# backtato/ai-video-detector

Hardware: AMD Instinct MI355X
Metric: sampled frames/sec analysed (1080p30 60 s clip, 2 fps sampling) (higher is better)
Workload: dtype u8 pixels; f32/f64 Farneback (cv2's own types); 1 GPU; BASELINE.json configs[1]: 1080p30 60 s clip, 2 fps sampling, one clip per GPU per step; frames_per_clip=120, height=1080, width=1920, clips_in_flight_per_gpu=3, fb_mode=fast+rerun, fb_wide160=2, parallelism=single GPU, rccl_ranks_seen=1

## Files before the change

### ai-video-detector_amd/csrc/avd_farneback.hip

```cpp
#include "avd_internal.h"
#include "avd_fb_device.h"

#pragma clang fp contract(off)

namespace {

constexpr int S = AVD_SMALL;

template <int K>
struct PyrGeo {
    static constexpr int WL = S >> K;
    static constexpr int NC = K == 0 ? S : 2 * WL;
    static constexpr int OFF = K == 0 ? 0 : (1 << K) / 2 - 1;
    static constexpr int TR = K >= 2 ? 4 : 8;
    static constexpr int TILES = WL / TR;
    static constexpr int KS = K == 3 ? 19 : (K == 2 ? 9 : 3), HALF = KS / 2;
    static constexpr int SROWS = K == 0 ? TR + 2 * HALF : ((TR - 1) << K) + 2 + 2 * HALF;
    static constexpr int PADX = 12, PS = S + 2 * PADX;
    static constexpr int SRC_BYTES = SROWS * PS, LDS_BYTES = SRC_BYTES + SROWS * NC * 4;
};
constexpr int cmax(int a, int b) { return a > b ? a : b; }
constexpr int cgcd(int a, int b) { return b == 0 ? a : cgcd(b, a % b); }

template <int PR>
// ... 22 lines not shown
    constexpr int WL = G::WL, NC = G::NC, OFF = G::OFF, TR = G::TR, KS = G::KS, HALF = G::HALF, SROWS = G::SROWS;
    constexpr int PADX = G::PADX, PS = G::PS;
    uint8_t (*src)[PS] = reinterpret_cast<uint8_t (*)[PS]>(lds);
    float (*rowf)[NC] = reinterpret_cast<float (*)[NC]>(lds + G::SRC_BYTES);
    const int tiles = WL / TR;
    const int f = blk / tiles, t = blk - f * tiles;
    const int tid = threadIdx.x;
    const int dy0 = t * TR;
    const int y_first = (K == 0 ? dy0 : (dy0 << K) + OFF) - HALF;
    const uint8_t* img = small + (int64_t)f * AVD_NPIX;
    const bool cmp = K == 1 && pairdiff != nullptr && f + 1 < n;
    int differs = 0;
    for (int it = tid; it < SROWS * (S / 4); it += 256) {
        const int r = it / (S / 4), c4 = it - r * (S / 4);
        const int y = reflect101(y_first + r, S);
        const unsigned v = reinterpret_cast<const unsigned*>(img + y * S)[c4];
        reinterpret_cast<unsigned*>(src[r] + PADX)[c4] = v;
        if (K == 1 && cmp) differs |= v != reinterpret_cast<const unsigned*>(img + AVD_NPIX + y * S)[c4];
    }
    for (int it = tid; it < SROWS * 2 * HALF; it += 256) {
        const int r = it / (2 * HALF), i = it - r * (2 * HALF);
        const uint8_t* g = img + reflect101(y_first + r, S) * S;
        if (i < HALF) src[r][PADX - 1 - i] = g[1 + i];
        else src[r][PADX + S + (i - HALF)] = g[S - 2 - (i - HALF)];
    }
    if (K == 1 && cmp) {
        const int any = __syncthreads_or(differs);
        if (tid == 0) pairdiff[f * tiles + t] = any;
    } else
        __syncthreads();
    float kw[KS];
#pragma unroll
    for (int q = 0; q < KS; q++) kw[q] = C->gk[K][q];
    if (KS == 3) {
        static_assert(KS != 3 || NC == S, "the 3-tap scales filter whole rows");
        using W = PyrWalk<S / 4>;
        typedef float f4 __attribute__((ext_vector_type(4)));
        const unsigned* wp0[W::PER]; f4* dst0[W::PER]; int r0[W::PER];
        {
            int r, c4;
            W::first(tid, r, c4);
#pragma unroll
            for (int i = 0; i < W::PER; i++) {
                r0[i] = r;
                wp0[i] = reinterpret_cast<const unsigned*>(src[r] + PADX + 4 * c4);
                dst0[i] = reinterpret_cast<f4*>(&rowf[r][4 * c4]);
                W::next(r, c4);
            }
        }
        for (int sb = 0; sb < SROWS; sb += W::SG) {
#pragma unroll
            for (int i = 0; i < W::PER; i++) {
                if (256 * i >= SROWS * (S / 4) || r0[i] + sb >= SROWS) continue;
                const unsigned* wp = wp0[i] + sb * (PS / 4);
                const unsigned pw = wp[-1], cwd = wp[0], nw = wp[1];
                const float b[6] = {(float)(pw >> 24), (float)(cwd & 0xFFu), (float)((cwd >> 8) & 0xFFu), (float)((cwd >> 16) & 0xFFu),
                                    (float)(cwd >> 24), (float)(nw & 0xFFu)};
                f4 o;
#pragma unroll
                for (int e = 0; e < 4; e++) o[e] = __builtin_fmaf(b[e + 1], kw[1], (b[e] + b[e + 2]) * kw[0]);
                dst0[i][sb * (NC / 4)] = o;
            }
        }
    } else {
        using W = PyrWalk<NC>;
        constexpr int NW = (KS + 3) / 4;
        const unsigned* wp0[W::PER]; float* dst0[W::PER]; int r0[W::PER], sh0[W::PER];
        {
            int r, j;
            W::first(tid, r, j);
#pragma unroll
            for (int i = 0; i < W::PER; i++) {
                const int x = K == 0 ? j : ((j >> 1) << K) + OFF + (j & 1);
                const int base = PADX + x - HALF;
                r0[i] = r; sh0[i] = base & 3;
                wp0[i] = reinterpret_cast<const unsigned*>(src[r] + (base & ~3));
                dst0[i] = &rowf[r][j];
                W::next(r, j);
            }
        }
        for (int sb = 0; sb < SROWS; sb += W::SG) {
#pragma unroll
            for (int i = 0; i < W::PER; i++) {
                if (256 * i >= SROWS * NC || r0[i] + sb >= SROWS) continue;
                const unsigned* wp = wp0[i] + sb * (PS / 4);
                unsigned d[NW + 1];
#pragma unroll
                for (int q = 0; q <= NW; q++) d[q] = wp[q];
                float v = 0.f;
#pragma unroll
                for (int q = 0; q < NW; q++) {
                    const unsigned wv = __builtin_amdgcn_alignbyte(d[q + 1], d[q], sh0[i]);
#pragma unroll
                    for (int e = 0; e < 4; e++)
                        if (q * 4 + e < KS) v = __builtin_fmaf((float)((wv >> (8 * e)) & 0xFFu), kw[q * 4 + e], v);
                }
                dst0[i][sb * NC] = v;
            }
        }
    }
    __syncthreads();
    auto colf = [&](const float* c) {
        float sacc = __builtin_fmaf(c[0], kw[HALF], 0.f);
#pragma unroll
        for (int k = 1; k <= HALF; k++) sacc = __builtin_fmaf(c[k * NC] + c[-k * NC], kw[HALF + k], sacc);
        return sacc;
    };
    {
        using W = PyrWalk<WL>;
        float* out = I + ((int64_t)f * WL + dy0) * WL;
        int dyl, dx;
        W::first(tid, dyl, dx);
#pragma unroll
        for (int i = 0; i < W::PER; i++) {
            if (256 * i < TR * WL) {
                for (int y = dyl; y < TR; y += W::SG) {
                    float o;
                    if (K == 0) {
                        o = colf(&rowf[y + HALF][dx]);
                    } else {
                        const float* c = &rowf[(y << K) + HALF][2 * dx];
                        const float p00 = colf(c), p01 = colf(c + 1);
                        const float p10 = colf(c + NC), p11 = colf(c + NC + 1);
                        o = ((p00 + p01) + (p10 + p11)) * 0.25f;
                    }
                    out[y * WL + dx] = o;
                }
            }
            W::next(dyl, dx);
        }
    }
}

__global__ __launch_bounds__(256) void k_pyramid_all(const uint8_t* __restrict__ small, int n, const FbConsts* __restrict__ C,
                                                    float* __restrict__ I0, float* __restrict__ I1, float* __restrict__ I2,
                                                    float* __restrict__ I3, int* __restrict__ flags, int* __restrict__ pairdiff)
{
    static_assert(PyrGeo<1>::TILES == kPairDiffTiles, "avd_fbfast.hip reads one word per 160-px tile");
    __shared__ __align__(16) char lds[kPyrLds];
    if (flags && (int)(blockIdx.x * 256 + threadIdx.x) < n - 1) flags[blockIdx.x * 256 + threadIdx.x] = 0;
    const int n3 = n * PyrGeo<3>::TILES, n2 = n * PyrGeo<2>::TILES, n1 = n * PyrGeo<1>::TILES;
    int b = blockIdx.x;
    if (b < n3) { pyramid_body<3>(lds, b, small, C, I3); return; }
    b -= n3;
    if (b < n2) { pyramid_body<2>(lds, b, small, C, I2); return; }
    b -= n2;
    if (b < n1) { pyramid_body<1>(lds, b, small, C, I1, n, pairdiff); return; }
    if (I0) pyramid_body<0>(lds, b - n1, small, C, I0);
}

struct PolyPtrs { const float* I[AVD_FB_LEVELS]; float* R[AVD_FB_LEVELS]; const uint8_t* small; };

constexpr int kPolyRows = 16;

template <bool FOLD>
__device__ __forceinline__ void polyexp_rows320(const float* __restrict__ img, const uint8_t* __restrict__ small, float* __restrict__ out, int y0,
                                                const FbConsts* __restrict__ C, float (*rowb)[3][S + 80], float (*outb)[S * 5])
{
    constexpr int w = S, h = S;
    const int x = threadIdx.x;
    const int xs = x - 1 < 0 ? 0 : (x - 1 > w - 4 ? w - 4 : x - 1);
    const int shl = ((x == 0 ? 1 : x - 1) - xs) * 8, shc = (x - xs) * 8, shr = ((x == w - 1 ? w - 2 : x + 1) - xs) * 8;
    const float kx0 = C->gk[0][0], kx1 = C->gk[0][1], kx2 = C->gk[0][2];
    struct __attribute__((packed, aligned(1))) U4 { unsigned v; };
    auto hb = [&](int srow) __attribute__((always_inline)) {
        const int sr = srow < 0 ? -srow : (srow > h - 1 ? 2 * (h - 1) - srow : srow);
        const unsigned wd = reinterpret_cast<const U4*>(small + sr * w + xs)->v;
        const float l = (float)((wd >> shl) & 0xFFu), c = (float)((wd >> shc) & 0xFFu), r = (float)((wd >> shr) & 0xFFu);
        return __builtin_fmaf(c, kx1, (l + r) * kx0);
    };
    float hm = 0.f, h0 = 0.f, hp = 0.f;
    int rcur = -1000;
    auto blurred = [&](int r) __attribute__((always_inline)) {
        if (r != rcur) {
            if (r == rcur + 1) { hm = h0; h0 = hp; hp = hb(r + 1); }
            else { hm = hb(r - 1); h0 = hb(r); hp = hb(r + 1); }
            rcur = r;
        }
        return __builtin_fmaf(hp + hm, kx2, __builtin_fmaf(h0, kx1, 0.f));
    };
    auto pixel = [&](int r) __attribute__((always_inline)) { return FOLD ? blurred(r) : img[r * w + x]; };
    typedef float f4 __attribute__((ext_vector_type(4)));
    typedef float f2 __attribute__((ext_vector_type(2)));
    float g[6], xg[6], xxg[6];
    double gd[6], xxgd[6];
#pragma unroll
    for (int q = 0; q <= 5; q++) { g[q] = C->g[5 + q]; xg[q] = C->xg[5 + q]; xxg[q] = C->xxg[5 + q]; gd[q] = (double)g[q]; xxgd[q] = (double)xxg[q]; }
    const double ig11 = C->ig11, ig03 = C->ig03, ig33 = C->ig33, ig55 = C->ig55;
    float win[11 + kPolyRows];
#pragma unroll
    for (int q = 0; q < 10; q++) win[q] = pixel(min(max(y0 - 5 + q, 0), h - 1));
#pragma unroll
    for (int i = 0; i < kPolyRows; i++) {
        const int y = y0 + i, par = i & 1;
        win[i + 10] = pixel(min(y + 5, h - 1));
        {
            f2 t02 = f2{win[i + 5] * g[0], 0.f};
            float t1 = 0.f;
#pragma unroll
            for (int q = 1; q <= 5; q++) {
                const float a = win[i + 5 - q], bb = win[i + 5 + q];
                const float p = a + bb;
                t02 = t02 + f2{g[q], xxg[q]} * f2{p, p};
                t1 = t1 + xg[q] * (bb - a);
            }
            float* r0s = rowb[par][0]; float* r1s = rowb[par][1]; float* r2s = rowb[par][2];
            const float t0 = t02.x, t2 = t02.y;
            r0s[x + 5] = t0; r1s[x + 5] = t1; r2s[x + 5] = t2;
            if (x == 0)
                for (int q = 0; q < 5; q++) { r0s[q] = t0; r1s[q] = t1; r2s[q] = t2; }
            if (x == w - 1)
                for (int q = 0; q < 5; q++) { r0s[w + 5 + q] = t0; r1s[w + 5 + q] = t1; r2s[w + 5 + q] = t2; }
        }
        __syncthreads();
        if (i > 0) {
            f4* dst = reinterpret_cast<f4*>(out + (int64_t)(y - 1) * w * 5);
            const f4* srcv = reinterpret_cast<const f4*>(outb[par ^ 1]);
            __builtin_nontemporal_store(srcv[x], dst + x);
            if (x < S * 5 / 4 - 320) __builtin_nontemporal_store(srcv[x + 320], dst + x + 320);
        }
        const float* r0 = rowb[par][0] + x + 5; const float* r1 = rowb[par][1] + x + 5; const float* r2 = rowb[par][2] + x + 5;
        double b1 = (double)(r0[0] * g[0]), b2 = 0, b3 = (double)(r1[0] * g[0]), b4 = 0, b5 = (double)(r2[0] * g[0]), b6 = 0;
#pragma unroll
        for (int q = 1; q <= 5; q++) {
            const float r0p = r0[q], r0m = r0[-q], r1p = r1[q], r1m = r1[-q], r2p = r2[q], r2m = r2[-q];
            const double tg = (double)(r0p + r0m);
            b1 = __builtin_fma(tg, gd[q], b1);
            b4 = __builtin_fma(tg, xxgd[q], b4);
            b2 += (double)((r0p - r0m) * xg[q]);
            b3 += (double)((r1p + r1m) * g[q]);
            b6 += (double)((r1p - r1m) * xg[q]);
            b5 += (double)((r2p + r2m) * g[q]);
        }
        float* o = outb[par] + x * 5;
        o[0] = (float)(b3 * ig11);
        o[1] = (float)(b2 * ig11);
        o[2] = (float)(b1 * ig03 + b5 * ig33);
        o[3] = (float)(b1 * ig03 + b4 * ig33);
        o[4] = (float)(b6 * ig55);
    }
    __syncthreads();
    {
        f4* dst = reinterpret_cast<f4*>(out + (int64_t)(y0 + kPolyRows - 1) * w * 5);
        const f4* srcv = reinterpret_cast<const f4*>(outb[(kPolyRows - 1) & 1]);
        __builtin_nontemporal_store(srcv[x], dst + x);
        if (x < S * 5 / 4 - 320) __builtin_nontemporal_store(srcv[x + 320], dst + x + 320);
    }
}

__global__ __launch_bounds__(320) void k_polyexp_all(PolyPtrs P, int n, const FbConsts* __restrict__ C)
{
    __shared__ float rowb[2][3][S + 80];
    __shared__ __align__(16) float outbb[2][S * 5];
    float (*row)[S + 80] = rowb[0];
    float* outb = outbb[0];
    {
        const int wgs0 = n * (S / kPolyRows), cnt0 = ((wgs0 + 7) >> 3) << 3;
        if ((int)blockIdx.x < cnt0) {
            const int per = cnt0 >> 3, lid = ((int)blockIdx.x & 7) * per + ((int)blockIdx.x >> 3);
            if (lid >= wgs0) return;
            const int f = lid / (S / kPolyRows), y0 = (lid - f * (S / kPolyRows)) * kPolyRows;
            if (P.small) polyexp_rows320<true>(nullptr, P.small + (int64_t)f * S * S, P.R[0] + (int64_t)f * S * S * 5, y0, C, rowb, outbb);
            else polyexp_rows320<false>(P.I[0] + (int64_t)f * S * S, nullptr, P.R[0] + (int64_t)f * S * S * 5, y0, C, rowb, outbb);
            return;
        }
    }
    int b = (int)blockIdx.x - ((((n * (S / kPolyRows)) + 7) >> 3) << 3), k = 1;
    for (; k < AVD_FB_LEVELS; k++) {
        const int cnt = ((n * (S >> (2 * k)) + 7) >> 3) << 3;
        if (b < cnt) break;
        b -= cnt;
    }
    if (k >= AVD_FB_LEVELS) return;
    const int wgs = n * (S >> (2 * k));
    const int per = ((wgs + 7) >> 3), lid = (b & 7) * per + (b >> 3);
    if (lid >= wgs) return;
    const int w = S >> k, h = w;
    const int wgs_per_frame = h >> k;
    const int f = lid / wgs_per_frame, y0 = (lid - f * wgs_per_frame) << k;
    const int tid = threadIdx.x;
    const int sr = tid / w, x = tid - sr * w;
    const int y = y0 + sr;
    const float* img = P.I[k] + (int64_t)f * w * h;
    const float* g = C->g + 5; const float* xg = C->xg + 5; const float* xxg = C->xxg + 5;
    const int pitch = w + 10;
    float* r0s = row[0] + sr * pitch; float* r1s = row[1] + sr * pitch; float* r2s = row[2] + sr * pitch;
    {
        float t0 = img[y * w + x] * g[0], t1 = 0.f, t2 = 0.f;
#pragma unroll
        for (int q = 1; q <= 5; q++) {
            const float a = img[max(y - q, 0) * w + x], bb = img[min(y + q, h - 1) * w + x];
            const float p = a + bb;
            t0 = t0 + g[q] * p;
            t1 = t1 + xg[q] * (bb - a);
            t2 = t2 + xxg[q] * p;
        }
        r0s[x + 5] = t0; r1s[x + 5] = t1; r2s[x + 5] = t2;
        if (x == 0)
            for (int q = 0; q < 5; q++) { r0s[q] = t0; r1s[q] = t1; r2s[q] = t2; }
        if (x == w - 1)
            for (int q = 0; q < 5; q++) { r0s[w + 5 + q] = t0; r1s[w + 5 + q] = t1; r2s[w + 5 + q] = t2; }
    }
    __syncthreads();
    const float* r0 = r0s + x + 5; const float* r1 = r1s + x + 5; const float* r2 = r2s + x + 5;
    double b1 = (double)(r0[0] * g[0]), b2 = 0, b3 = (double)(r1[0] * g[0]), b4 = 0,
           b5 = (double)(r2[0] * g[0]), b6 = 0;
#pragma unroll
    for (int q = 1; q <= 5; q++) {
        const double tg = (double)(r0[q] + r0[-q]);
        b1 = __builtin_fma(tg, (double)g[q], b1);
        b4 = __builtin_fma(tg, (double)xxg[q], b4);
        b2 += (double)((r0[q] - r0[-q]) * xg[q]);
        b3 += (double)((r1[q] + r1[-q]) * g[q]);
        b6 += (double)((r1[q] - r1[-q]) * xg[q]);
        b5 += (double)((r2[q] + r2[-q]) * g[q]);
    }
    float* o = outb + tid * 5;
    o[0] = (float)(b3 * C->ig11);
    o[1] = (float)(b2 * C->ig11);
    o[2] = (float)(b1 * C->ig03 + b5 * C->ig33);
    o[3] = (float)(b1 * C->ig03 + b4 * C->ig33);
    o[4] = (float)(b6 * C->ig55);
    __syncthreads();
    typedef float f4 __attribute__((ext_vector_type(4)));
    f4* dst = reinterpret_cast<f4*>(P.R[k] + ((int64_t)f * w * h + (int64_t)y0 * w) * 5);
    const f4* srcv = reinterpret_cast<const f4*>(outb);
    __builtin_nontemporal_store(srcv[tid], dst + tid);
    if (tid < S * 5 / 4 - 320) __builtin_nontemporal_store(srcv[tid + 320], dst + tid + 320);
}

template <int W>
__global__ __launch_bounds__(256) void k_flow_up(const float* __restrict__ prev, float* __restrict__ flow, int npairs, const int* __restrict__ plist)
{
    constexpr int H = W, PW = W / 2, PH = H / 2, Q = W / 4;
    const int gid = blockIdx.x * 256 + threadIdx.x;
    if (gid >= npairs * 2 * H * Q) return;
    const int q = gid % Q;
    const int dy = (gid / Q) % H;
    int pc = gid / (Q * H);
    if (plist) pc = plist[pc >> 1] * 2 + (pc & 1);
    const float* src = prev + (int64_t)pc * PW * PH;
    float fy = dy * 0.5f - 0.25f;
    const int sy = floor_f(fy);
    fy -= sy;
    const float* r0 = src + clampi(sy, 0, PH - 1) * PW;
    const float* r1 = src + clampi(sy + 1, 0, PH - 1) * PW;
    const float b0 = 1.f - fy, b1 = fy;
    float o[4];
#pragma unroll
    for (int i = 0; i < 4; i++) {
        const int dx = q * 4 + i;
        float fx = dx * 0.5f - 0.25f;
        int sx = floor_f(fx);
        fx -= sx;
        if (sx < 0) { fx = 0; sx = 0; }
        bool edge = false;
        if (sx + 1 >= PW) { edge = true; if (sx >= PW - 1) { fx = 0; sx = PW - 1; } }
        const int x1 = min(sx + 1, PW - 1);
        const float a0 = 1.f - fx, a1 = fx;
        float d0, d1;
        if (edge) { d0 = r0[sx] * 1.f; d1 = r1[sx] * 1.f; }
        else { d0 = r0[sx] * a0 + r0[x1] * a1; d1 = r1[sx] * a0 + r1[x1] * a1; }
        o[i] = (d0 * b0 + d1 * b1) * 2.f;
    }
    *reinterpret_cast<float4*>(flow + ((int64_t)pc * H + dy) * W + q * 4) = make_float4(o[0], o[1], o[2], o[3]);
}

constexpr int kChunk = 8192;
constexpr int kNChunk = (AVD_NPIX + kChunk - 1) / kChunk;

__device__ __forceinline__ float chunk_total(const float* part)
{
    float t = part[0];
#pragma unroll
    for (int i = 1; i < kNChunk; i++) t += part[i];
    return t;
}

__global__ __launch_bounds__(512) void k_stats_pair(const float* __restrict__ mag, float* __restrict__ stats, const int* __restrict__ plist)
{
    __shared__ float wpart[kNChunk][8];
    __shared__ float ctot[kNChunk];
    const int p = plist ? plist[blockIdx.x] : (int)blockIdx.x, tid = threadIdx.x;
    const int l = tid >> 3, wave = tid >> 6;
    const bool in_last = l < ((AVD_NPIX - (kNChunk - 1) * kChunk) >> 7);
    const float* src = mag + (int64_t)p * AVD_NPIX + l * 128 + (tid & 7);
    float v[kNChunk][16];
#pragma unroll
    for (int c = 0; c < kNChunk; c++)
#pragma unroll
        for (int k = 0; k < 16; k++) v[c][k] = (c < kNChunk - 1 || in_last) ? src[c * kChunk + 8 * k] : 0.f;
    float total[2];
#pragma unroll
    for (int pass = 0; pass < 2; pass++) {
#pragma unroll
        for (int c = 0; c < kNChunk; c++) {
            float r = v[c][0];
#pragma unroll
            for (int k = 1; k < 16; k++) r += v[c][k];
#pragma unroll
            for (int d = 1; d < 64; d <<= 1) r = r + __shfl_down(r, d);
            if ((tid & 63) == 0) wpart[c][wave] = r;
        }
        __syncthreads();
        if (tid < kNChunk) {
            const float* w = wpart[tid];
            ctot[tid] = tid < kNChunk - 1 ? ((w[0] + w[1]) + (w[2] + w[3])) + ((w[4] + w[5]) + (w[6] + w[7])) : (w[0] + w[1]) + (w[2] + w[3]);
        }
        __syncthreads();
        total[pass] = chunk_total(ctot);
        if (pass == 0) {
            const float mean32 = total[0] / (float)AVD_NPIX;
#pragma unroll
            for (int c = 0; c < kNChunk; c++)
#pragma unroll
                for (int k = 0; k < 16; k++) { const float d = v[c][k] - mean32; v[c][k] = d * d; }
            __syncthreads();
        }
    }
    if (tid == 0) {
        stats[2 * p] = (float)((double)total[0] / (double)AVD_NPIX);
        stats[2 * p + 1] = (float)((double)total[1] / (double)AVD_NPIX);
    }
}

__global__ void k_mag(const float* __restrict__ flow, float* __restrict__ mag, int64_t total4, const int* __restrict__ plist)
{
    const int64_t gid = (int64_t)blockIdx.x * 256 + threadIdx.x;
    if (gid >= total4) return;
    const int64_t ps = gid / (AVD_NPIX / 4), i = gid - ps * (AVD_NPIX / 4);
    const int64_t p = plist ? plist[ps] : ps;
    const float4 fx = reinterpret_cast<const float4*>(flow + p * 2 * AVD_NPIX)[i], fy = reinterpret_cast<const float4*>(flow + (p * 2 + 1) * AVD_NPIX)[i];
    float4 m;
    m.x = sqrtf(fx.x * fx.x + fy.x * fy.x);
    m.y = sqrtf(fx.y * fx.y + fy.y * fy.y);
    m.z = sqrtf(fx.z * fx.z + fy.z * fy.z);
    m.w = sqrtf(fx.w * fx.w + fy.w * fy.w);
    reinterpret_cast<float4*>(mag + p * AVD_NPIX)[i] = m;
}

__global__ void k_flow_interleave(const float* __restrict__ flow, float* __restrict__ out, int64_t total)
{
    const int64_t gid = (int64_t)blockIdx.x * 256 + threadIdx.x;
    if (gid >= total) return;
    const int64_t p = gid / AVD_NPIX, i = gid - p * AVD_NPIX;
    out[gid * 2] = flow[p * 2 * AVD_NPIX + i];
    out[gid * 2 + 1] = flow[(p * 2 + 1) * AVD_NPIX + i];
}

template <typename... A>
inline void launch1d(void (*k)(A...), int64_t items, int block, hipStream_t s, A... args)
{
    const int grid = (int)((items + block - 1) / block);
    if (grid > 0) hipLaunchKernelGGL(k, dim3(grid), dim3(block), 0, s, args...);
}

constexpr int kLevelId[AVD_FB_LEVELS] = {AVD_K_LEVEL320, AVD_K_LEVEL160, AVD_K_LEVEL80, AVD_K_LEVEL40};
constexpr int kFlowUpId[AVD_FB_LEVELS - 1] = {AVD_K_FLOWUP320, AVD_K_FLOWUP160, AVD_K_FLOWUP80};

void pyramid_and_polyexp(avd_ctx* ctx, const uint8_t* d_small, int n)
{
    Workspace& ws = ctx->ws;
    const FbConsts* C = ctx->d_fbc;
    const bool fold = ctx->fb_fold_blur != 0;
    const int wgs = n * ((fold ? 0 : PyrGeo<0>::TILES) + PyrGeo<1>::TILES + PyrGeo<2>::TILES + PyrGeo<3>::TILES);
    kmark(ctx, AVD_K_PYRAMID);
    hipLaunchKernelGGL(k_pyramid_all, dim3(wgs), dim3(256), 0, ctx->stream, d_small, n, C, fold ? nullptr : ws.d_pyr[0].p, ws.d_pyr[1].p, ws.d_pyr[2].p,
                       ws.d_pyr[3].p, ws.d_fbflags.p, ws.d_pairdiff.p);
    PolyPtrs P;
    P.small = fold ? d_small : nullptr;
    int grid = ((n * (S / kPolyRows) + 7) >> 3) << 3;
    for (int k = 0; k < AVD_FB_LEVELS; k++) {
        P.I[k] = ws.d_pyr[k]; P.R[k] = ws.d_poly[k];
        if (k > 0) grid += ((n * (S >> (2 * k)) + 7) >> 3) << 3;
    }
    kmark(ctx, AVD_K_POLYEXP);
    hipLaunchKernelGGL(k_polyexp_all, dim3(grid), dim3(320), 0, ctx->stream, P, n, C);
}

void flow_up_level(hipStream_t stream, int k, const float* prev, float* flow, int np, const int* plist)
{
    fb_dispatch_width(S >> k, [&](auto wc) {
        constexpr int W = decltype(wc)::value;
        if constexpr (W > S / 8) launch1d(k_flow_up<W>, (int64_t)np * 2 * W * (W / 4), 256, stream, prev, flow, np, plist);
    });
}

int exact_levels(avd_ctx* ctx, int np, int fused_mask, FbTwoScratch scratch, const int* plist)
{
    Workspace& ws = ctx->ws;
    const hipStream_t stream = ctx->stream;
    const bool rerun = plist != nullptr;
    float* const flow0 = rerun ? const_cast<float*>(ws.flow_res[0]) : ws.d_flow[0].p;
    if (rerun) kmark(ctx, AVD_K_RERUN);
    for (int k = AVD_FB_LEVELS - 1; k >= 0; k--) {
        const int w = S >> k;
        const bool coarsest = k == AVD_FB_LEVELS - 1, fused = (fused_mask >> k) & 1;
        float* flow = k == 0 ? flow0 : ws.d_flow[k].p;
        if (coarsest) {
            if (!fused && rerun) { ctx->err = "exact re-run: the coarsest level runs the fused kernel (it needs no cleared flow)"; return AVD_ERR_ARG; }
            if (!fused) HIP_TRY(ctx, hipMemsetAsync(flow, 0, sizeof(float) * 2 * w * w * np, stream));
        } else {
            if (!rerun) kmark(ctx, kFlowUpId[k]);
            flow_up_level(stream, k, ws.d_flow[k + 1], flow, np, plist);
        }
        if (!rerun) { ws.flow_res[k] = flow; kmark(ctx, kLevelId[k]); }
        const bool marks = !rerun && k == 0;
        if (fused) {
            stage_mark(ctx, marks);
            if (int e = launch_fb_level(ctx, stream, w, ws.d_poly[k], flow, np, 3, coarsest, plist)) return e;
            stage_mark(ctx, marks);
        } else {
            for (int it = 0; it < 3; it++)
                if (int e = launch_fb_two(ctx, stream, w, ws.d_poly[k], flow, scratch, np, plist, marks)) return e;
        }
    }
    return 0;
}

int fast_levels(avd_ctx* ctx, int np)
{
    Workspace& ws = ctx->ws;
    const hipStream_t stream = ctx->stream;
    const int fold = ctx->fb_fold_up;
    int* flags = ctx->fb_rerun ? ws.d_fbflags.p : nullptr;
    const int* pairdiff = ctx->fb_rerun ? ws.d_pairdiff.p : nullptr;
    for (int k = AVD_FB_LEVELS - 1; k >= 0; k--) {
        const int w = S >> k;
        const bool coarsest = k == AVD_FB_LEVELS - 1, three = (k == 2 || k == 3) && (fold & 4);
        float *a = ws.d_flow[k], *b = ws.d_flow2[k];
        const float* prev = coarsest ? nullptr : ws.flow_res[k + 1];
        const bool chain = (k == 0 && (fold & 1)) || (k == 1 && ctx->fb_fold_up160 && ctx->fb_wide160_used);
        const FbFlowFrom from = coarsest ? FbFlowFrom::zero : chain ? FbFlowFrom::chain
                                : ((k == 1 || k == 2) && (fold & 2)) ? FbFlowFrom::prologue : FbFlowFrom::level;
        if (from == FbFlowFrom::level) {
            kmark(ctx, kFlowUpId[k]);
            flow_up_level(stream, k, prev, a, np, nullptr);
        }
        const bool from_prev = from == FbFlowFrom::chain || from == FbFlowFrom::prologue;
        kmark(ctx, kLevelId[k]);
        stage_mark(ctx, k == 0);
        if (three) {
            const FbFastLaunch L{3, from, from_prev ? prev : a, b, a, nullptr, flags, pairdiff};
            if (int e = launch_fb_fast(ctx, stream, w, ws.d_poly[k], L, np)) return e;
            a = b;
        } else {
            for (int it = 0; it < 3; it++) {
                float* mag = (k == 0 && it == 2) ? ws.d_mag.p : nullptr;
                const FbFastLaunch L{1, it == 0 ? from : FbFlowFrom::level, it == 0 && from_prev ? prev : a, b, a, mag, flags, pairdiff};
                if (int e = launch_fb_fast(ctx, stream, w, ws.d_poly[k], L, np)) return e;
                float* t = a; a = b; b = t;
            }
        }
        stage_mark(ctx, k == 0);
        ws.flow_res[k] = a;
    }
    return 0;
}

void flow_tail(avd_ctx* ctx, const float* flow, bool with_mag, int m, const int* plist, int np_chunk)
{
    Workspace& ws = ctx->ws;
    const hipStream_t stream = ctx->stream;
    if (with_mag) launch1d(k_mag, (int64_t)m * (AVD_NPIX / 4), 256, stream, flow, ws.d_mag.p, (int64_t)m * (AVD_NPIX / 4), plist);
    hipLaunchKernelGGL(k_stats_pair, dim3(m), dim3(512), 0, stream, (const float*)ws.d_mag, ws.d_stats.p, plist);
    if (!ws.no_flow_il && ws.d_flow_il)
        launch1d(k_flow_interleave, (int64_t)np_chunk * AVD_NPIX, 256, stream, flow, ws.d_flow_il.p, (int64_t)np_chunk * AVD_NPIX);
}

}

int launch_farneback(avd_ctx* ctx, const uint8_t* d_small, int n)
{
    if (n < 2) return 0;
    Workspace& ws = ctx->ws;
    if (ctx->profiling) ctx->kern_ev_used = 0;
    const bool fast = ctx->fb_mode == 1;
    ws.mag_valid = fast;
    pyramid_and_polyexp(ctx, d_small, n);
    if (int e = fast ? fast_levels(ctx, n - 1) : exact_levels(ctx, n - 1, ctx->fb_fused, {ws.d_vs, ws.d_vs0}, nullptr)) return e;
    HIP_TRY(ctx, hipGetLastError());
    return 0;
}

int launch_farneback_rerun(avd_ctx* ctx, const int* h_list, int m, int np_chunk)
{
    if (m <= 0) return 0;
    Workspace& ws = ctx->ws;
    if (m > ws.fb_cap) { ctx->err = "re-run list longer than the chunk"; return AVD_ERR_ARG; }
    if (int e = ws.d_rlist.reserve(ctx, (size_t)ws.fb_cap)) return e;
    const int fused_mask = m <= kRerunTwoKernelMax ? (ctx->fb_rerun_fused & 0xF) : 0xF;
    if (fused_mask != 0xF) {
        const FbTwoScratchSize sz = fb_two_scratch_size(kRerunTwoKernelMax);
        if (int e = ws.d_vs0_rerun.reserve(ctx, sz.vs0)) return e;
        if (int e = ws.d_vs_rerun.reserve(ctx, sz.vs)) return e;
    }
    HIP_TRY(ctx, hipMemcpyAsync(ws.d_rlist, h_list, sizeof(int) * m, hipMemcpyHostToDevice, ctx->stream));
    if (int e = exact_levels(ctx, m, fused_mask, {ws.d_vs_rerun, ws.d_vs0_rerun}, ws.d_rlist)) return e;
    flow_tail(ctx, ws.flow_res[0], true, m, ws.d_rlist, np_chunk);
    HIP_TRY(ctx, hipGetLastError());
    return 0;
}

int launch_flow_stats(avd_ctx* ctx, int n)
{
    if (n < 2) return 0;
    Workspace& ws = ctx->ws;
    kmark(ctx, AVD_K_STATS);
    flow_tail(ctx, ws.flow_res[0] ? ws.flow_res[0] : ws.d_flow[0].p, !ws.mag_valid, n - 1, nullptr, n - 1);
    HIP_TRY(ctx, hipGetLastError());
    return 0;
}
```

### ai-video-detector_amd/csrc/avd_internal.h

```cpp
#pragma once
#include <hip/hip_runtime.h>
#include <stdint.h>
#include <mutex>
#include <string>
#include <type_traits>
#include <vector>
#include "../../include/avd.h"
#include "avd_ingest_clip.h"

#define AVD_FB_LEVELS 4
#define AVD_NPIX (AVD_SMALL * AVD_SMALL)
constexpr int kPairDiffTiles = 20;

#define HIP_TRY(ctx, expr)                                                         \
    do {                                                                           \
        hipError_t e__ = (expr);                                                   \
        if (e__ != hipSuccess) {                                                   \
            (ctx)->err = std::string(#expr) + ": " + hipGetErrorString(e__);       \
            return AVD_ERR_DEVICE;                                                 \
        }                                                                          \
    } while (0)

struct LinearTab {
    std::vector<int> x0, x1, y0, y1;
    std::vector<short> a0, a1, b0, b1;
};
void build_linear_tab(int src_h, int src_w, int dst_h, int dst_w, LinearTab& t);

struct AreaAxis {
    std::vector<int> begin, count;
    std::vector<float> w_first, w_mid, w_last;
};
struct AreaTab {
    AreaAxis x, y;
    int fast;
    int iscale_x, iscale_y;
};
int build_area_tab(int src_h, int src_w, int dst_h, int dst_w, AreaTab& t);

struct FbConsts {
    float g[11], xg[11], xxg[11];
    double ig11, ig03, ig33, ig55;
    float gk[AVD_FB_LEVELS][19];
    int gksize[AVD_FB_LEVELS];
};
void build_fb_consts(FbConsts& c);

struct YuvConsts { int cy, crv, cbu, cgu, cgv, c0, kr, kb, kg, bias, ntab; };
void build_yuv_consts(YuvConsts& c, bool full_range);
void yuv_index_window(const YuvConsts& c, int& lo, int& hi);

struct LinTap { short i0, i1, w0, w1; };

struct PreParams {
    const LinTap *lxt, *lyt;
    const int* band_dy;
    const int *ax_begin, *ax_count;
    const float *ax_first, *ax_mid, *ax_last;
    int area_fast;
    int area_x_uniform4;
    int h, w, rows_per_band, nbands, pitch;
    int64_t row_stride, frame_stride;
};

struct HashParams {
    const int *ay_begin, *ay_count;
    const float *ay_first, *ay_mid, *ay_last;
    int area_fast, fast_area, fast_simd_w;
    int h;
};

struct BandPlan { int rows_per_band, pitch, ni; };
BandPlan band_plan(int w);
enum IngestKernel { kIngestBgrScalar = 0, kIngestBgrVec16, kIngestBgrStaged, kIngestNv12Scalar, kIngestNv12Tables, kIngestI420Scalar, kIngestI420Tables,
                    kIngestNv12Strip, kIngestI420Strip, kIngestPx32Scalar, kIngestPx32Vec16, kIngestRgbpScalar, kIngestRgbpVec16, kIngestRgbpStaged,
                    kIngestYuyvScalar, kIngestYuyvTables, kIngestI422Scalar, kIngestI422Tables, kIngestNv16Scalar, kIngestNv16Tables,
                    kIngestP010Scalar, kIngestP010Tables, kIngestI010Scalar, kIngestI010Tables, kIngestP010Strip, kIngestI010Strip };
static_assert(kIngestP010Scalar == 20 && kIngestI010Strip == 25, "the ids include/avd.h lists");
struct IngestPlan { int h, w, rows_per_band, nbands, pitch, ni, lds_bytes, kernel; };
static_assert(sizeof(IngestPlan) == 8 * sizeof(int), "avd_debug_fetch hands the struct out as int32[8]");
struct IngestRecord {
    IngestPlan plan{};
    int launched = 0;
    int32_t rotate = 0;
    int32_t range = 0;
    int32_t format = 0;
    int32_t list[2] = {0, 0};
    int64_t stage_copies = -1;
    int64_t stage_bytes = -1;
};
enum CnnShape { kCnnFolded = 0, kCnn128x128, kCnn256x64, kCnn256x128, kCnn256x256, kCnnStem, kCnnConv3Expand, kCnnSlab3Expand };
constexpr int kCnnConvs = 53;
constexpr int kCnnTapImage = 1, kCnnTapConv0 = 2, kCnnTapMaxPool = kCnnTapConv0 + kCnnConvs, kCnnTapPooled = kCnnTapMaxPool + 1;
constexpr int kLapSlots = 8;

struct avd_ctx;
template <typename T, bool kPinned>
struct Buf {
    T* p = nullptr;
    size_t cap = 0;
    Buf() = default;
    Buf(const Buf&) = delete;
    Buf& operator=(const Buf&) = delete;
    Buf(Buf&& o) noexcept : p(o.p), cap(o.cap) { o.p = nullptr; o.cap = 0; }
    Buf& operator=(Buf&& o) noexcept
    {
        if (this != &o) { reset(); p = o.p; cap = o.cap; o.p = nullptr; o.cap = 0; }
        return *this;
    }
    ~Buf() { reset(); }
    void reset()
    {
        if (p) { if (kPinned) (void)hipHostFree(p); else (void)hipFree(p); }
        p = nullptr; cap = 0;
    }
    int reserve(avd_ctx* ctx, size_t count);
    operator T*() const { return p; }
};
template <typename T> using DevBuf = Buf<T, false>;
template <typename T> using PinBuf = Buf<T, true>;

constexpr int kGeomCache = 4;
struct Geom {
    int h = 0, w = 0;
    DevBuf<uint8_t> d_tables;
    PreParams pre{};
    HashParams hsh{};
    unsigned long long stamp = 0;
};

struct Workspace {
    int cap_n = 0;
    Geom geoms[kGeomCache];
    unsigned long long geom_clock = 0;
    int f0 = 0; size_t rowbuf_off = 0, lappart_off = 0;
    int fb_cap = 0;
    DevBuf<int> d_clipstart; PinBuf<int> h_clipstart;
    DevBuf<uint8_t> d_stage;
    DevBuf<const uint8_t*> d_ftab; PinBuf<const uint8_t*> h_ftab;
    DevBuf<uint8_t> d_small;
    DevBuf<float> d_rowbuf;
    DevBuf<uint8_t> d_area;
    DevBuf<uint8_t> d_hash;
    DevBuf<unsigned long long> d_lap;
    DevBuf<long long> d_lap_part;
    PreParams pre{};
    HashParams hsh{};
    DevBuf<float> d_pyr[AVD_FB_LEVELS];
    DevBuf<float> d_poly[AVD_FB_LEVELS];
    DevBuf<float> d_flow[AVD_FB_LEVELS];
    DevBuf<float> d_flow2[AVD_FB_LEVELS];
    const float* flow_res[AVD_FB_LEVELS] = {};
    DevBuf<float> d_mag;
    int mag_valid = 0;
    DevBuf<int> d_fbflags;
    DevBuf<int> d_pairdiff;
    DevBuf<int> d_rlist;
    PinBuf<int> h_rlist;
    DevBuf<double> d_vs_rerun, d_vs0_rerun;
    DevBuf<double> d_vs;
    DevBuf<double> d_vs0;
    DevBuf<float> d_flow_il;
    int no_flow_il = 0;
    DevBuf<float> d_stats;
    DevBuf<avd_frame_record> d_rec;
    PinBuf<avd_frame_record> h_rec;
    DevBuf<uint16_t> d_vit_patches;
    DevBuf<float> d_vit_tokens;
    DevBuf<double> d_audio_tab; int audio_win = 0, audio_last = 0;
    DevBuf<double> d_audio_buf;
    DevBuf<avd_audio_window> d_audio_out;
    DevBuf<uint16_t> d_cnn_act[4], d_cnn_img;
    DevBuf<float> d_cnn_pool, d_cnn_logits; int cnn_frames = 0;
    DevBuf<uint16_t> d_cnn_tap;
    int cnn_tap_asked = 0, cnn_tap_point = 0;
    size_t cnn_tap_rows = 0, cnn_tap_bytes = 0;
    int cnn_tap_c = 0;
};

struct Weights {
    DevBuf<uint16_t> d_cnn_w; DevBuf<float> d_cnn_b;
    std::vector<size_t> cnn_w_off; size_t cnn_fc_off = 0;
    DevBuf<uint16_t> d_vit_w; DevBuf<float> d_vit_bias; int vit_has_bias = 0;
};

struct avd_ctx {
    int device = 0;
    int num_cus = 256;
    hipStream_t stream = nullptr;
    hipEvent_t ev0 = nullptr, ev1 = nullptr;
    hipEvent_t ev_in = nullptr;
    avd_frame_record* pending_out = nullptr;
    int pending_n = 0;
    hipEvent_t stage_ev[5] = {};
    hipEvent_t kern_ev[12] = {};
    int kern_ev_used = 0;
    int profiling = 0;
// ... 127 lines not shown
```

### ai-video-detector_amd/csrc/avd_tables.cpp

```cpp
#include <cfloat>
#include <climits>
#include <cmath>
#include <cstring>
#include "avd_internal.h"

namespace {

inline int round_half_even(double v) { return (int)std::nearbyint(v); }
inline int round_half_even(float v) { return (int)std::nearbyintf(v); }
inline int floor_i(float v) { int i = (int)v; return i - (i > v); }
inline int floor_i(double v) { int i = (int)v; return i - (i > v); }
inline int ceil_i(double v) { int i = (int)v; return i + (i < v); }
inline short to_q11(float v) {
    int i = round_half_even(v * 2048.f);
    return (short)std::min(32767, std::max(-32768, i));
}
inline int clamp_idx(int v, int n) { return v < 0 ? 0 : (v >= n ? n - 1 : v); }

void linear_axis(int src, int dst, bool snap_weights_at_edges, std::vector<int>& i0,
                 std::vector<int>& i1, std::vector<short>& w0, std::vector<short>& w1)
{
    const double scale = 1. / ((double)dst / src);
    i0.resize(dst); i1.resize(dst); w0.resize(dst); w1.resize(dst);
    for (int d = 0; d < dst; d++) {
        float f = (float)((d + 0.5) * scale - 0.5);
        int s = floor_i(f);
        f -= s;
        if (snap_weights_at_edges) {
            if (s < 0) { f = 0; s = 0; }
            if (s >= src - 1) { f = 0; s = src - 1; }
        }
        w0[d] = to_q11(1.f - f);
        w1[d] = to_q11(f);
        i0[d] = clamp_idx(s, src);
        i1[d] = clamp_idx(s + 1, src);
    }
}

void area_axis(int src, int dst, double scale, AreaAxis& ax)
{
    ax.begin.assign(dst, 0); ax.count.assign(dst, 0);
    ax.w_first.assign(dst, 0.f); ax.w_mid.assign(dst, 0.f); ax.w_last.assign(dst, 0.f);
    for (int d = 0; d < dst; d++) {
        const double lo = d * scale, hi = lo + scale;
        const double cell = std::min(scale, src - lo);
        int s1 = ceil_i(lo), s2 = floor_i(hi);
        s2 = std::min(s2, src - 1);
        s1 = std::min(s1, s2);
        std::vector<float> wts;
        int first = s1;
        if (s1 - lo > 1e-3) { first = s1 - 1; wts.push_back((float)((s1 - lo) / cell)); }
        for (int s = s1; s < s2; s++) wts.push_back((float)(1.0 / cell));
        if (hi - s2 > 1e-3) wts.push_back((float)(std::min(std::min(hi - s2, 1.), cell) / cell));
        ax.begin[d] = first;
        ax.count[d] = (int)wts.size();
        if (!wts.empty()) {
            ax.w_first[d] = wts.front();
            ax.w_last[d] = wts.back();
            ax.w_mid[d] = wts.size() > 2 ? wts[1] : wts.front();
        }
    }
}

}

void build_linear_tab(int src_h, int src_w, int dst_h, int dst_w, LinearTab& t)
{
    linear_axis(src_w, dst_w, true, t.x0, t.x1, t.a0, t.a1);
    linear_axis(src_h, dst_h, false, t.y0, t.y1, t.b0, t.b1);
}

int build_area_tab(int src_h, int src_w, int dst_h, int dst_w, AreaTab& t)
{
    const double sx = 1. / ((double)dst_w / src_w), sy = 1. / ((double)dst_h / src_h);
    if (!(sx >= 1 && sy >= 1)) return AVD_ERR_UNSUPPORTED;
    t.iscale_x = round_half_even(sx);
    t.iscale_y = round_half_even(sy);
    t.fast = std::fabs(sx - t.iscale_x) < DBL_EPSILON && std::fabs(sy - t.iscale_y) < DBL_EPSILON;
    area_axis(src_w, dst_w, sx, t.x);
    area_axis(src_h, dst_h, sy, t.y);
    return 0;
}

namespace {

void gaussian_taps(int n, double sigma, float* k)
{
    if (sigma <= 0 && n == 3) { k[0] = 0.25f; k[1] = 0.5f; k[2] = 0.25f; return; }
    const double sig = sigma > 0 ? sigma : std::fma((double)n, 0.15, 0.35);
    const double scale2 = -0.125 / (sig * sig);
    const int half = (n - 1) / 2;
    double v[32];
    double sum = 0;
    for (int i = 0, x = 1 - n; i < half; i++, x += 2) {
        v[i] = std::exp((double)(x * x) * scale2);
        sum += v[i];
    }
    sum *= 2;
    sum += 1;
    const double norm = 1. / sum;
    for (int i = 0; i < half; i++) k[i] = k[n - 1 - i] = (float)(v[i] * norm);
    k[half] = (float)(1. * norm);
}

void spd_inverse6(double A[6][6], double X[6][6])
{
    for (int i = 0; i < 6; i++) {
        for (int j = 0; j < i; j++) {
            double s = A[i][j];
            for (int k = 0; k < j; k++) s -= A[i][k] * A[j][k];
            A[i][j] = s * A[j][j];
        }
        double s = A[i][i];
        for (int k = 0; k < i; k++) { double t = A[i][k]; s -= t * t; }
        A[i][i] = 1. / std::sqrt(s);
    }
    for (int i = 0; i < 6; i++)
        for (int j = 0; j < 6; j++) {
            double s = X[i][j];
            for (int k = 0; k < i; k++) s -= A[i][k] * X[k][j];
            X[i][j] = s * A[i][i];
        }
    for (int i = 5; i >= 0; i--)
        for (int j = 0; j < 6; j++) {
            double s = X[i][j];
            for (int k = 5; k > i; k--) s -= A[k][i] * X[k][j];
            X[i][j] = s * A[i][i];
        }
}

}

void build_fb_consts(FbConsts& c)
{
    std::memset(&c, 0, sizeof c);
    const int n = 5;
    const double sigma = 1.2;
    float* g = c.g + n; float* xg = c.xg + n; float* xxg = c.xxg + n;
    double s = 0.;
    for (int x = -n; x <= n; x++) {
        g[x] = (float)std::exp(-x * x / (2 * sigma * sigma));
        s += g[x];
    }
    s = 1. / s;
    for (int x = -n; x <= n; x++) {
        g[x] = (float)(g[x] * s);
        xg[x] = (float)(x * g[x]);
        xxg[x] = (float)(x * x * g[x]);
    }
    double G[6][6] = {}, inv[6][6] = {};
    for (int y = -n; y <= n; y++)
        for (int x = -n; x <= n; x++) {
            const float gg = g[y] * g[x];
            G[0][0] += gg;
            G[1][1] += gg * x * x;
            G[3][3] += gg * x * x * x * x;
            G[5][5] += gg * x * x * y * y;
        }
    G[2][2] = G[0][3] = G[0][4] = G[3][0] = G[4][0] = G[1][1];
    G[4][4] = G[3][3];
    G[3][4] = G[4][3] = G[5][5];
    for (int i = 0; i < 6; i++) inv[i][i] = 1.;
    spd_inverse6(G, inv);
    c.ig11 = inv[1][1]; c.ig03 = inv[0][3]; c.ig33 = inv[3][3]; c.ig55 = inv[5][5];

    for (int k = 0; k < AVD_FB_LEVELS; k++) {
        double scale = 1;
        for (int i = 0; i < k; i++) scale *= 0.5;
        const double sig = (1. / scale - 1) * 0.5;
        int ks = round_half_even(sig * 5) | 1;
        ks = std::max(ks, 3);
        c.gksize[k] = ks;
        gaussian_taps(ks, sig, c.gk[k]);
    }
}

void build_yuv_consts(YuvConsts& c, bool full_range)
{
    const long long one = 1ll << 16;
    const long long cy = full_range ? one : one * 255 / 219;
    const long long oy = full_range ? 0 : 16ll << 16;
    auto ranged = [&](long long inc) { return full_range ? inc * 224 / 255 : inc; };
    auto rescale = [&](long long inc) { return (inc * one + 0x8000) / cy; };
    const long long crv = rescale(ranged(104597)), cbu = rescale(ranged(132201)), cgu = rescale(ranged(-25675)), cgv = rescale(ranged(-53279));
    auto fl = [](long long v, int s) { return v >= 0 ? v >> s : -((-v + (1ll << s) - 1) >> s); };
    c.cy = (int)cy; c.crv = (int)crv; c.cbu = (int)cbu; c.cgu = (int)cgu; c.cgv = (int)cgv;
    c.c0 = (int)(-(384ll << 16) - oy + (full_range ? 384 : 326) * cy + 0x8000);
    c.kr = (int)-fl(crv, 9);
    c.kb = (int)-fl(cbu, 9);
    c.kg = (int)(-fl(cgu, 9) - fl(cgv, 9));
    c.bias = full_range ? 228 : 224;
    c.ntab = full_range ? 712 : 704;
}

void yuv_index_window(const YuvConsts& c, int& lo, int& hi)
{
    auto term = [](int s, int coef) { return (int)(((long long)s * coef) >> 16); };
    int rmin = INT_MAX, rmax = INT_MIN, bmin = INT_MAX, bmax = INT_MIN, gumin = INT_MAX, gumax = INT_MIN, gvmin = INT_MAX, gvmax = INT_MIN;
    for (int s = 0; s < 256; s++) {
        rmin = std::min(rmin, term(s, c.crv)); rmax = std::max(rmax, term(s, c.crv));
        bmin = std::min(bmin, term(s, c.cbu)); bmax = std::max(bmax, term(s, c.cbu));
        gumin = std::min(gumin, term(s, c.cgu)); gumax = std::max(gumax, term(s, c.cgu));
        gvmin = std::min(gvmin, term(s, c.cgv)); gvmax = std::max(gvmax, term(s, c.cgv));
    }
    lo = std::min({rmin + c.kr, bmin + c.kb, gumin + gvmin + c.kg});
    hi = std::max({rmax + c.kr, bmax + c.kb, gumax + gvmax + c.kg}) + 255;
}
```

Before: 139,400 frames/s.

## Generalize row-walking polynomial expansion to levels 1-2 with packed LDS quads

The polynomial expansion kernel's row-walking 16-row band path, previously used only at the 320-px scale, now also serves pyramid levels 1 and 2. Several image rows are processed per step in one workgroup with a sliding vertical window, so levels 1 and 2 now run as 16-row bands instead of the old per-level row grouping, which should cut redundant vertical reads and workgroup count. The LDS row buffers change from three separate float planes to interleaved float4 quads, so each horizontal tap is one vector LDS read. Double-precision tap constants are precomputed on the host. The cost is more complex indexing and possibly higher register pressure at the coarser levels.

```diff
diff --git a/ai-video-detector_amd/csrc/avd_farneback.hip b/ai-video-detector_amd/csrc/avd_farneback.hip
--- a/ai-video-detector_amd/csrc/avd_farneback.hip
+++ b/ai-video-detector_amd/csrc/avd_farneback.hip
@@ -198,13 +198,59 @@
 struct PolyPtrs { const float* I[AVD_FB_LEVELS]; float* R[AVD_FB_LEVELS]; const uint8_t* small; };
 
 constexpr int kPolyRows = 16;
-
-template <bool FOLD>
-__device__ __forceinline__ void polyexp_rows320(const float* __restrict__ img, const uint8_t* __restrict__ small, float* __restrict__ out, int y0,
-                                                const FbConsts* __restrict__ C, float (*rowb)[3][S + 80], float (*outb)[S * 5])
-{
-    constexpr int w = S, h = S;
-    const int x = threadIdx.x;
+constexpr int kPolyQuads = 4 * (S / 4 + 10);
+static_assert(AVD_FB_LEVELS == 4, "three walking scales and the one-row form of the coarsest");
+__host__ __device__ constexpr int poly_wgs(int k) { return k < AVD_FB_LEVELS - 1 ? (S >> k) / kPolyRows : S >> (2 * k); }
+
+typedef float pf4 __attribute__((ext_vector_type(4)));
+typedef float pf2 __attribute__((ext_vector_type(2)));
+
+__device__ __forceinline__ void polyexp_put(pf4* __restrict__ rowq, int x, int w, float t0, float t1, float t2)
+{
+    const pf4 t = {t0, t1, t1, t2};
+    rowq[x + 5] = t;
+    if (x == 0)
+        for (int q = 0; q < 5; q++) rowq[q] = t;
+    if (x == w - 1)
+        for (int q = 0; q < 5; q++) rowq[w + 5 + q] = t;
+}
+
+__device__ __forceinline__ void polyexp_hpass(const pf4* __restrict__ rq, const float (&g)[6], const float (&xg)[6], const double (&gd)[6],
+                                              const double (&xxgd)[6], double ig11, double ig03, double ig33, double ig55, float* __restrict__ o)
+{
+    const pf4 c = rq[0];
+    double b1 = (double)(c.x * g[0]), b2 = 0, b3 = (double)(c.y * g[0]), b4 = 0, b5 = (double)(c.w * g[0]), b6 = 0;
+#pragma unroll
+    for (int q = 1; q <= 5; q++) {
+        const pf4 p = rq[q], m = rq[-q];
+        const pf2 s01 = p.xy + m.xy, d01 = p.xy - m.xy, s12 = p.zw + m.zw;
+        const pf2 dx = d01 * pf2{xg[q], xg[q]};
+        const pf2 sg = s12 * pf2{g[q], g[q]};
+        const double tg = (double)s01.x;
+        b1 = __builtin_fma(tg, gd[q], b1);
+        b4 = __builtin_fma(tg, xxgd[q], b4);
+        b2 += (double)dx.x;
+        b3 += (double)sg.x;
+        b6 += (double)dx.y;
+        b5 += (double)sg.y;
+    }
+    o[0] = (float)(b3 * ig11);
+    o[1] = (float)(b2 * ig11);
+    o[2] = (float)(b1 * ig03 + b5 * ig33);
+    o[3] = (float)(b1 * ig03 + b4 * ig33);
+    o[4] = (float)(b6 * ig55);
+}
+
+template <int K, bool FOLD>
+__device__ __forceinline__ void polyexp_rows(const float* __restrict__ img, const uint8_t* __restrict__ small, float* __restrict__ out, int y0,
+                                             const FbConsts* __restrict__ C, pf4 (*rowb)[kPolyQuads], float (*outb)[S * 5])
+{
+    static_assert(!FOLD || K == 0, "only the 320-px scale forms its own blur");
+    constexpr int w = S >> K, h = w, R = 1 << K, STEPS = kPolyRows / R;
+    static_assert(R * (w + 10) <= kPolyQuads && h % kPolyRows == 0 && kPolyRows % R == 0, "a step's R rows fit one LDS buffer; whole bands");
+    const int tid = threadIdx.x;
+    const int sr = K == 0 ? 0 : tid / w, x = tid - sr * w;
+    const int yb = y0 + sr;
     const int xs = x - 1 < 0 ? 0 : (x - 1 > w - 4 ? w - 4 : x - 1);
     const int shl = ((x == 0 ? 1 : x - 1) - xs) * 8, shc = (x - xs) * 8, shr = ((x == w - 1 ? w - 2 : x + 1) - xs) * 8;
     const float kx0 = C->gk[0][0], kx1 = C->gk[0][1], kx2 = C->gk[0][2];
@@ -231,106 +277,89 @@
     float g[6], xg[6], xxg[6];
     double gd[6], xxgd[6];
 #pragma unroll
-    for (int q = 0; q <= 5; q++) { g[q] = C->g[5 + q]; xg[q] = C->xg[5 + q]; xxg[q] = C->xxg[5 + q]; gd[q] = (double)g[q]; xxgd[q] = (double)xxg[q]; }
+    for (int q = 0; q <= 5; q++) { g[q] = C->g[5 + q]; xg[q] = C->xg[5 + q]; xxg[q] = C->xxg[5 + q]; gd[q] = C->gd[q]; xxgd[q] = C->xxgd[q]; }
     const double ig11 = C->ig11, ig03 = C->ig03, ig33 = C->ig33, ig55 = C->ig55;
-    float win[11 + kPolyRows];
-#pragma unroll
-    for (int q = 0; q < 10; q++) win[q] = pixel(min(max(y0 - 5 + q, 0), h - 1));
-#pragma unroll
-    for (int i = 0; i < kPolyRows; i++) {
-        const int y = y0 + i, par = i & 1;
-        win[i + 10] = pixel(min(y + 5, h - 1));
+    float win[11 + kPolyRows - R];
+#pragma unroll
+    for (int q = 0; q < 10; q++) win[q] = pixel(min(max(yb - 5 + q, 0), h - 1));
+    pf4* rowq[2] = {rowb[0] + sr * (w + 10), rowb[1] + sr * (w + 10)};
+#pragma unroll
+    for (int i = 0; i < STEPS; i++) {
+        const int par = i & 1, o = R * i;
+#pragma unroll
+        for (int j = o + 11 - R; j <= o + 10; j++)
+            if (j >= 10) win[j] = pixel(min(yb - 5 + j, h - 1));
         {
-            f2 t02 = f2{win[i + 5] * g[0], 0.f};
+            f2 t02 = f2{win[o + 5] * g[0], 0.f};
             float t1 = 0.f;
 #pragma unroll
             for (int q = 1; q <= 5; q++) {
-                const float a = win[i + 5 - q], bb = win[i + 5 + q];
+                const float a = win[o + 5 - q], bb = win[o + 5 + q];
                 const float p = a + bb;
                 t02 = t02 + f2{g[q], xxg[q]} * f2{p, p};
                 t1 = t1 + xg[q] * (bb - a);
             }
-            float* r0s = rowb[par][0]; float* r1s = rowb[par][1]; float* r2s = rowb[par][2];
-            const float t0 = t02.x, t2 = t02.y;
-            r0s[x + 5] = t0; r1s[x + 5] = t1; r2s[x + 5] = t2;
-            if (x == 0)
-                for (int q = 0; q < 5; q++) { r0s[q] = t0; r1s[q] = t1; r2s[q] = t2; }
-            if (x == w - 1)
-                for (int q = 0; q < 5; q++) { r0s[w + 5 + q] = t0; r1s[w + 5 + q] = t1; r2s[w + 5 + q] = t2; }
+            polyexp_put(rowq[par], x, w, t02.x, t1, t02.y);
         }
         __syncthreads();
         if (i > 0) {
-            f4* dst = reinterpret_cast<f4*>(out + (int64_t)(y - 1) * w * 5);
+            f4* dst = reinterpret_cast<f4*>(out + (int64_t)(y0 + o - R) * w * 5);
             const f4* srcv = reinterpret_cast<const f4*>(outb[par ^ 1]);
-            __builtin_nontemporal_store(srcv[x], dst + x);
-            if (x < S * 5 / 4 - 320) __builtin_nontemporal_store(srcv[x + 320], dst + x + 320);
-        }
-        const float* r0 = rowb[par][0] + x + 5; const float* r1 = rowb[par][1] + x + 5; const float* r2 = rowb[par][2] + x + 5;
-        double b1 = (double)(r0[0] * g[0]), b2 = 0, b3 = (double)(r1[0] * g[0]), b4 = 0, b5 = (double)(r2[0] * g[0]), b6 = 0;
-#pragma unroll
-        for (int q = 1; q <= 5; q++) {
-            const float r0p = r0[q], r0m = r0[-q], r1p = r1[q], r1m = r1[-q], r2p = r2[q], r2m = r2[-q];
-            const double tg = (double)(r0p + r0m);
-            b1 = __builtin_fma(tg, gd[q], b1);
-            b4 = __builtin_fma(tg, xxgd[q], b4);
-            b2 += (double)((r0p - r0m) * xg[q]);
-            b3 += (double)((r1p + r1m) * g[q]);
-            b6 += (double)((r1p - r1m) * xg[q]);
-            b5 += (double)((r2p + r2m) * g[q]);
-        }
-        float* o = outb[par] + x * 5;
-        o[0] = (float)(b3 * ig11);
-        o[1] = (float)(b2 * ig11);
-        o[2] = (float)(b1 * ig03 + b5 * ig33);
-        o[3] = (float)(b1 * ig03 + b4 * ig33);
-        o[4] = (float)(b6 * ig55);
+            __builtin_nontemporal_store(srcv[tid], dst + tid);
+            if (tid < S * 5 / 4 - 320) __builtin_nontemporal_store(srcv[tid + 320], dst + tid + 320);
+        }
+        polyexp_hpass(rowq[par] + x + 5, g, xg, gd, xxgd, ig11, ig03, ig33, ig55, outb[par] + tid * 5);
     }
     __syncthreads();
     {
-        f4* dst = reinterpret_cast<f4*>(out + (int64_t)(y0 + kPolyRows - 1) * w * 5);
-        const f4* srcv = reinterpret_cast<const f4*>(outb[(kPolyRows - 1) & 1]);
-        __builtin_nontemporal_store(srcv[x], dst + x);
-        if (x < S * 5 / 4 - 320) __builtin_nontemporal_store(srcv[x + 320], dst + x + 320);
+        f4* dst = reinterpret_cast<f4*>(out + (int64_t)(y0 + kPolyRows - R) * w * 5);
+        const f4* srcv = reinterpret_cast<const f4*>(outb[(STEPS - 1) & 1]);
+        __builtin_nontemporal_store(srcv[tid], dst + tid);
+        if (tid < S * 5 / 4 - 320) __builtin_nontemporal_store(srcv[tid + 320], dst + tid + 320);
     }
 }
 
 __global__ __launch_bounds__(320) void k_polyexp_all(PolyPtrs P, int n, const FbConsts* __restrict__ C)
 {
-    __shared__ float rowb[2][3][S + 80];
+    __shared__ pf4 rowb[2][kPolyQuads];
     __shared__ __align__(16) float outbb[2][S * 5];
-    float (*row)[S + 80] = rowb[0];
+    pf4* row = rowb[0];
+    static_assert(8 * (S / 8 + 10) <= 2 * kPolyQuads, "the eight sub-rows of the coarsest scale fit");
     float* outb = outbb[0];
-    {
-        const int wgs0 = n * (S / kPolyRows), cnt0 = ((wgs0 + 7) >> 3) << 3;
-        if ((int)blockIdx.x < cnt0) {
-            const int per = cnt0 >> 3, lid = ((int)blockIdx.x & 7) * per + ((int)blockIdx.x >> 3);
-            if (lid >= wgs0) return;
-            const int f = lid / (S / kPolyRows), y0 = (lid - f * (S / kPolyRows)) * kPolyRows;
-            if (P.small) polyexp_rows320<true>(nullptr, P.small + (int64_t)f * S * S, P.R[0] + (int64_t)f * S * S * 5, y0, C, rowb, outbb);
-            else polyexp_rows320<false>(P.I[0] + (int64_t)f * S * S, nullptr, P.R[0] + (int64_t)f * S * S * 5, y0, C, rowb, outbb);
-            return;
-        }
-    }
-    int b = (int)blockIdx.x - ((((n * (S / kPolyRows)) + 7) >> 3) << 3), k = 1;
+    int b = (int)blockIdx.x, k = 0, wgs = 0;
     for (; k < AVD_FB_LEVELS; k++) {
-        const int cnt = ((n * (S >> (2 * k)) + 7) >> 3) << 3;
+        wgs = n * poly_wgs(k);
+        const int cnt = ((wgs + 7) >> 3) << 3;
         if (b < cnt) break;
         b -= cnt;
     }
     if (k >= AVD_FB_LEVELS) return;
-    const int wgs = n * (S >> (2 * k));
-    const int per = ((wgs + 7) >> 3), lid = (b & 7) * per + (b >> 3);
+    const int per = (wgs + 7) >> 3, lid = (b & 7) * per + (b >> 3);
     if (lid >= wgs) return;
     const int w = S >> k, h = w;
-    const int wgs_per_frame = h >> k;
-    const int f = lid / wgs_per_frame, y0 = (lid - f * wgs_per_frame) << k;
+    int f = 0;
+#pragma unroll
+    for (int kk = 0; kk < AVD_FB_LEVELS; kk++)
+        if (k == kk) f = lid / poly_wgs(kk);
+    const int t = lid - f * poly_wgs(k);
+    float* R = P.R[k] + (int64_t)f * w * h * 5;
+    if (k == 0) {
+        if (P.small) polyexp_rows<0, true>(nullptr, P.small + (int64_t)f * S * S, R, t * kPolyRows, C, rowb, outbb);
+        else polyexp_rows<0, false>(P.I[0] + (int64_t)f * S * S, nullptr, R, t * kPolyRows, C, rowb, outbb);
+        return;
+    }
+    if (k == 1) { polyexp_rows<1, false>(P.I[1] + (int64_t)f * w * h, nullptr, R, t * kPolyRows, C, rowb, outbb); return; }
+    if (k == 2) { polyexp_rows<2, false>(P.I[2] + (int64_t)f * w * h, nullptr, R, t * kPolyRows, C, rowb, outbb); return; }
+    const int y0 = t << k;
     const int tid = threadIdx.x;
     const int sr = tid / w, x = tid - sr * w;
     const int y = y0 + sr;
     const float* img = P.I[k] + (int64_t)f * w * h;
-    const float* g = C->g + 5; const float* xg = C->xg + 5; const float* xxg = C->xxg + 5;
-    const int pitch = w + 10;
-    float* r0s = row[0] + sr * pitch; float* r1s = row[1] + sr * pitch; float* r2s = row[2] + sr * pitch;
+    float g[6], xg[6], xxg[6];
+    double gd[6], xxgd[6];
+#pragma unroll
+    for (int q = 0; q <= 5; q++) { g[q] = C->g[5 + q]; xg[q] = C->xg[5 + q]; xxg[q] = C->xxg[5 + q]; gd[q] = C->gd[q]; xxgd[q] = C->xxgd[q]; }
+    pf4* rowq = row + sr * (w + 10);
     {
         float t0 = img[y * w + x] * g[0], t1 = 0.f, t2 = 0.f;
 #pragma unroll
@@ -341,35 +370,13 @@
             t1 = t1 + xg[q] * (bb - a);
             t2 = t2 + xxg[q] * p;
         }
-        r0s[x + 5] = t0; r1s[x + 5] = t1; r2s[x + 5] = t2;
-        if (x == 0)
-            for (int q = 0; q < 5; q++) { r0s[q] = t0; r1s[q] = t1; r2s[q] = t2; }
-        if (x == w - 1)
-            for (int q = 0; q < 5; q++) { r0s[w + 5 + q] = t0; r1s[w + 5 + q] = t1; r2s[w + 5 + q] = t2; }
+        polyexp_put(rowq, x, w, t0, t1, t2);
     }
     __syncthreads();
-    const float* r0 = r0s + x + 5; const float* r1 = r1s + x + 5; const float* r2 = r2s + x + 5;
-    double b1 = (double)(r0[0] * g[0]), b2 = 0, b3 = (double)(r1[0] * g[0]), b4 = 0,
-           b5 = (double)(r2[0] * g[0]), b6 = 0;
-#pragma unroll
-    for (int q = 1; q <= 5; q++) {
-        const double tg = (double)(r0[q] + r0[-q]);
-        b1 = __builtin_fma(tg, (double)g[q], b1);
-        b4 = __builtin_fma(tg, (double)xxg[q], b4);
-        b2 += (double)((r0[q] - r0[-q]) * xg[q]);
-        b3 += (double)((r1[q] + r1[-q]) * g[q]);
-        b6 += (double)((r1[q] - r1[-q]) * xg[q]);
-        b5 += (double)((r2[q] + r2[-q]) * g[q]);
-    }
-    float* o = outb + tid * 5;
-    o[0] = (float)(b3 * C->ig11);
-    o[1] = (float)(b2 * C->ig11);
-    o[2] = (float)(b1 * C->ig03 + b5 * C->ig33);
-    o[3] = (float)(b1 * C->ig03 + b4 * C->ig33);
-    o[4] = (float)(b6 * C->ig55);
+    polyexp_hpass(rowq + x + 5, g, xg, gd, xxgd, C->ig11, C->ig03, C->ig33, C->ig55, outb + tid * 5);
     __syncthreads();
     typedef float f4 __attribute__((ext_vector_type(4)));
-    f4* dst = reinterpret_cast<f4*>(P.R[k] + ((int64_t)f * w * h + (int64_t)y0 * w) * 5);
+    f4* dst = reinterpret_cast<f4*>(R + (int64_t)y0 * w * 5);
     const f4* srcv = reinterpret_cast<const f4*>(outb);
     __builtin_nontemporal_store(srcv[tid], dst + tid);
     if (tid < S * 5 / 4 - 320) __builtin_nontemporal_store(srcv[tid + 320], dst + tid + 320);
@@ -515,10 +522,10 @@
                        ws.d_pyr[3].p, ws.d_fbflags.p, ws.d_pairdiff.p);
     PolyPtrs P;
     P.small = fold ? d_small : nullptr;
-    int grid = ((n * (S / kPolyRows) + 7) >> 3) << 3;
+    int grid = 0;
     for (int k = 0; k < AVD_FB_LEVELS; k++) {
         P.I[k] = ws.d_pyr[k]; P.R[k] = ws.d_poly[k];
-        if (k > 0) grid += ((n * (S >> (2 * k)) + 7) >> 3) << 3;
+        grid += ((n * poly_wgs(k) + 7) >> 3) << 3;
     }
     kmark(ctx, AVD_K_POLYEXP);
     hipLaunchKernelGGL(k_polyexp_all, dim3(grid), dim3(320), 0, ctx->stream, P, n, C);
diff --git a/ai-video-detector_amd/csrc/avd_internal.h b/ai-video-detector_amd/csrc/avd_internal.h
--- a/ai-video-detector_amd/csrc/avd_internal.h
+++ b/ai-video-detector_amd/csrc/avd_internal.h
@@ -43,6 +43,7 @@
     double ig11, ig03, ig33, ig55;
     float gk[AVD_FB_LEVELS][19];
     int gksize[AVD_FB_LEVELS];
+    double gd[6], xxgd[6];
 };
 void build_fb_consts(FbConsts& c);
 
diff --git a/ai-video-detector_amd/csrc/avd_tables.cpp b/ai-video-detector_amd/csrc/avd_tables.cpp
--- a/ai-video-detector_amd/csrc/avd_tables.cpp
+++ b/ai-video-detector_amd/csrc/avd_tables.cpp
@@ -148,6 +148,7 @@
         xg[x] = (float)(x * g[x]);
         xxg[x] = (float)(x * x * g[x]);
     }
+    for (int q = 0; q <= n; q++) { c.gd[q] = (double)g[q]; c.xxgd[q] = (double)xxg[q]; }
     double G[6][6] = {}, inv[6][6] = {};
     for (int y = -n; y <= n; y++)
         for (int x = -n; x <= n; x++) {
```

Measured after the change: 140,900 frames/s (median of 6 runs). 1.1% higher.
